# Janspiry/Image-Super-Resolution-via-Iterative-Refinement

Measured on NVIDIA H100. Metric: diffusion steps/sec (batch16, 16->128 SR3), higher is better.
Workload: dtype bf16

## Files before the change

image-super-resolution-via-iterative-refinement_b200/csrc/attn_wgmma.cuh:

```cuda
#pragma once
#include <cuda_bf16.h>
#include <cuda.h>
#include "gemm_wgmma.cuh"

namespace sr3 {

constexpr int ATTN_THREADS = 288;
constexpr int ATTN_PRODUCER_WARP = 8;
constexpr int ATTN_STAGES = 3;
constexpr int ATTN_STAGE_BYTES = 16384 + 32768;
constexpr int ATTN_P_BYTES = 65536;
constexpr int ATTN_SMEM_BYTES = 1024 + GEMM_HDR_BYTES + ATTN_STAGES * ATTN_STAGE_BYTES + ATTN_P_BYTES;

struct AttnParams {
    CUtensorMap qk_map;
    CUtensorMap vt_map;
    __nv_bfloat16* out;
    int C, Lt, HW, dn, nz;
    float scale_log2e;
};

template <int LT, int DN>
__device__ __forceinline__ void attn_unit_t(const AttnParams& p, const AttnParams* pm, const uint32_t base_in, uint8_t* base_ptr_in,
                                            const int qt, const int dc, const int z) {
    const uint32_t bar_base = base_in;
    const uint32_t base = base_in + GEMM_HDR_BYTES;
    uint8_t* base_ptr = base_ptr_in + GEMM_HDR_BYTES;
    const uint32_t p_base = base + ATTN_STAGES * ATTN_STAGE_BYTES;
    uint8_t* p_ptr = base_ptr + ATTN_STAGES * ATTN_STAGE_BYTES;
    auto full_bar = [&](int s) { return bar_base + 8u * s; };
    auto empty_bar = [&](int s) { return bar_base + 8u * (ATTN_STAGES + s); };

    const int warp = threadIdx.x >> 5;
    const int lane = threadIdx.x & 31;
    const int kc1 = p.C / 64;
    constexpr int kc3 = LT / 64;

    if (threadIdx.x == 0) {
        tma_prefetch_desc(&pm->qk_map);
        tma_prefetch_desc(&pm->vt_map);
        for (int s = 0; s < ATTN_STAGES; ++s) { mbar_init(full_bar(s), 1); mbar_init(empty_bar(s), 2); }
        fence_mbar_init();
    }
    __syncthreads();
    pdl_launch_dependents();
    pdl_wait();

    if (warp == ATTN_PRODUCER_WARP) {
        int s = 0;
        uint32_t ph = 0;
        for (int it = 0; it < kc1 + kc3; ++it) {
            mbar_wait(empty_bar(s), ph ^ 1u);
            if (elect_one_sync()) {
                const uint32_t dst = base + s * ATTN_STAGE_BYTES;
                if (it < kc1) {
                    mbar_arrive_expect_tx(full_bar(s), 16384 + LT * 128);
                    tma_load_2d(dst, &pm->qk_map, full_bar(s), it * 64, z * LT + qt * 128);
                    for (int j = 0; j < LT / 128; ++j)
                        tma_load_2d(dst + 16384 + j * 16384, &pm->qk_map, full_bar(s), p.C + it * 64, z * LT + j * 128);
                } else {
                    mbar_arrive_expect_tx(full_bar(s), DN * 128);
                    for (int j = 0; j < DN / 128; ++j)
                        tma_load_2d(dst + 16384 + j * 16384, &pm->vt_map, full_bar(s), (it - kc1) * 64, z * p.C + dc * DN + j * 128);
                }
            }
            __syncwarp();
            if (++s == ATTN_STAGES) { s = 0; ph ^= 1u; }
        }
    } else if (warp < ATTN_PRODUCER_WARP) {
        const int g = warp >> 2;
        const int wq = warp & 3;
        const bool leader = (threadIdx.x & 127) == 0;
        int s = 0, prev = -1;
        uint32_t ph = 0;
        auto release_prev = [&]() {
            if (prev >= 0) {
                wgmma_wait<1>();
                mbar_arrive_if(empty_bar(prev), leader);
            }
            prev = s;
            if (++s == ATTN_STAGES) { s = 0; ph ^= 1u; }
        };
        float sacc[LT / 2];
        for (int it = 0; it < kc1; ++it) {
            mbar_wait(full_bar(s), ph);
            wgmma_fence();
            const uint32_t st = base + s * ATTN_STAGE_BYTES;
#pragma unroll
            for (int kk = 0; kk < 4; ++kk)
                Wgmma<LT>::template mma<0, 0>(sacc, wgmma_desc_sw128(st + g * 8192 + kk * 32, 16, 1024), wgmma_desc_sw128(st + 16384 + kk * 32, 16, 1024),
                                              (it | kk) != 0);
            wgmma_commit();
            release_prev();
        }
        wgmma_wait<0>();
        wgmma_fence_regs(sacc);
        int rows[2], segs[2];
        float mx[2] = {-3.0e38f, -3.0e38f}, sum[2] = {0.f, 0.f};
#pragma unroll
        for (int h = 0; h < 2; ++h) {
            rows[h] = 64 * g + 16 * wq + (lane >> 2) + 8 * h;
            segs[h] = (qt * 128 + rows[h]) / p.HW;
        }
#pragma unroll
        for (int j = 0; j < LT / 2; ++j) {
            const int h = (j >> 1) & 1, key = 8 * (j >> 2) + 2 * (lane & 3) + (j & 1);
            if (key / p.HW == segs[h]) mx[h] = fmaxf(mx[h], sacc[j]);
        }
#pragma unroll
        for (int h = 0; h < 2; ++h) {
            mx[h] = fmaxf(mx[h], __shfl_xor_sync(0xffffffffu, mx[h], 1));
            mx[h] = fmaxf(mx[h], __shfl_xor_sync(0xffffffffu, mx[h], 2));
        }
        const float mxs[2] = {mx[0] * p.scale_log2e, mx[1] * p.scale_log2e};
#pragma unroll
        for (int j = 0; j < LT / 2; j += 2) {
            const int h = (j >> 1) & 1, key = 8 * (j >> 2) + 2 * (lane & 3);
            const float x0 = exp2f(fmaf(sacc[j], p.scale_log2e, -mxs[h])), x1 = exp2f(fmaf(sacc[j + 1], p.scale_log2e, -mxs[h]));
            const float e0 = (key / p.HW == segs[h]) ? x0 : 0.f, e1 = ((key + 1) / p.HW == segs[h]) ? x1 : 0.f;
            sum[h] += e0 + e1;
            const int r = rows[h];
            uint8_t* dst = p_ptr + (key >> 6) * 16384 + (r >> 3) * 1024 + (r & 7) * 128 + ((((key & 63) >> 3) ^ (r & 7)) << 4) + (key & 7) * 2;
            *reinterpret_cast<__nv_bfloat162*>(dst) = __floats2bfloat162_rn(e0, e1);
        }
#pragma unroll
        for (int h = 0; h < 2; ++h) {
            sum[h] += __shfl_xor_sync(0xffffffffu, sum[h], 1);
            sum[h] += __shfl_xor_sync(0xffffffffu, sum[h], 2);
        }
        fence_proxy_async_smem();
        asm volatile("bar.sync %0, 128;" ::"r"(2 + g) : "memory");

        float oacc[DN / 2];
        for (int kc = 0; kc < kc3; ++kc) {
            mbar_wait(full_bar(s), ph);
            wgmma_fence();
            const uint32_t st = base + s * ATTN_STAGE_BYTES;
            const uint32_t pa = p_base + kc * 16384 + g * 8192;
#pragma unroll
            for (int kk = 0; kk < 4; ++kk)
                Wgmma<DN>::template mma<0, 0>(oacc, wgmma_desc_sw128(pa + kk * 32, 16, 1024), wgmma_desc_sw128(st + 16384 + kk * 32, 16, 1024),
                                              (kc | kk) != 0);
            wgmma_commit();
            release_prev();
        }
        wgmma_wait<0>();
        wgmma_fence_regs(oacc);
        if (prev >= 0) mbar_arrive_if(empty_bar(prev), leader);
        const float inv[2] = {1.0f / sum[0], 1.0f / sum[1]};
#pragma unroll
        for (int j = 0; j < DN / 2; j += 2) {
            const int h = (j >> 1) & 1, col = 8 * (j >> 2) + 2 * (lane & 3);
            __nv_bfloat16* o = p.out + (static_cast<long long>(z) * LT + qt * 128 + rows[h]) * p.C + dc * DN + col;
            *reinterpret_cast<__nv_bfloat162*>(o) = __floats2bfloat162_rn(oacc[j] * inv[h], oacc[j + 1] * inv[h]);
        }
    }
    __syncthreads();
}

__device__ __forceinline__ void attn_unit(const AttnParams& p, const AttnParams* pm, const uint32_t base, uint8_t* base_ptr, const int qt,
                                          const int dc, const int z) {
    if (p.Lt == 256) {
        if (p.dn == 256) attn_unit_t<256, 256>(p, pm, base, base_ptr, qt, dc, z);
        else attn_unit_t<256, 128>(p, pm, base, base_ptr, qt, dc, z);
    } else {
        if (p.dn == 256) attn_unit_t<128, 256>(p, pm, base, base_ptr, qt, dc, z);
        else attn_unit_t<128, 128>(p, pm, base, base_ptr, qt, dc, z);
    }
}

__global__ void __launch_bounds__(ATTN_THREADS, 1) attn_kernel(const __grid_constant__ AttnParams p) {
    extern __shared__ uint8_t smem_raw[];
    const uint32_t raw = smem_u32(smem_raw);
    const uint32_t base = (raw + 1023u) & ~1023u;
    const int n_dc = p.C / p.dn;
    attn_unit(p, &p, base, smem_raw + (base - raw), blockIdx.x / n_dc, blockIdx.x % n_dc, blockIdx.y);
}

}
```

image-super-resolution-via-iterative-refinement_b200/csrc/engine.cu:

```cuda
#include <cuda.h>
#include <cuda_runtime.h>

#include <cmath>
#include <cstdarg>
#include <cstdlib>
#include <cstring>
#include <functional>
#include <limits>
#include <map>
#include <memory>
#include <mutex>
#include <stdexcept>
#include <string>
#include <vector>

#include "../../include/sr3_b200.h"
#include "aux_kernels.cuh"
#include "attn_wgmma.cuh"
#include "attn_long_wgmma.cuh"
#include "train_kernels.cuh"
#include "window_kernels.cuh"
#include "stream_kernels.cuh"

using namespace sr3;
// ... 122 lines not shown
    if (s < 1) s = 1;
    return s;
}
int current_device() { int dev = 0; CK(cudaGetDevice(&dev)); return dev; }
int num_sms() {
    static std::map<int, int> cache;
    static std::mutex mu;
    std::lock_guard<std::mutex> lock(mu);
    const int dev = current_device();
    auto it = cache.find(dev);
    if (it != cache.end()) return it->second;
    int n = 0;
    CK(cudaDeviceGetAttribute(&n, cudaDevAttrMultiProcessorCount, dev));
    cache[dev] = n;
    return n;
}
bool first_use_on_device(std::vector<int>& seen) {
    static std::mutex mu;
    std::lock_guard<std::mutex> lock(mu);
    const int dev = current_device();
    for (int d : seen) if (d == dev) return false;
    seen.push_back(dev);
    return true;
}
template <typename... KArgs, typename... Args>
void launch_k(void (*kernel)(KArgs...), dim3 grid, dim3 block, size_t smem, cudaStream_t st, Args&&... args) {
    cudaLaunchConfig_t cfg{};
    cfg.gridDim = grid; cfg.blockDim = block; cfg.dynamicSmemBytes = smem; cfg.stream = st;
    cudaLaunchAttribute attr[1];
    attr[0].id = cudaLaunchAttributeProgrammaticStreamSerialization;
    attr[0].val.programmaticStreamSerializationAllowed = 1;
    cfg.attrs = attr; cfg.numAttrs = 1;
    CK(cudaLaunchKernelEx(&cfg, kernel, std::forward<Args>(args)...));
}
constexpr int MAX_CLUSTER_SPLIT = 8;
template <int BN, int MH, bool PP = false>
void launch_gemm_bn(const GemmParams& p, dim3 grid, int smem, cudaStream_t st) {
    if (p.ksplit == 1) { launch_k(gemm_tile_kernel<BN, MH, PP>, grid, dim3(GEMM_THREADS), (size_t)smem, st, p); return; }
    REQUIRE(!PP, "a ping-pong tile launch cannot be split");
    REQUIRE(p.ksplit <= MAX_CLUSTER_SPLIT && grid.x % p.ksplit == 0, "split-K factor %d does not form clusters of grid %u", p.ksplit, grid.x);
    cudaLaunchConfig_t cfg{};
    cfg.gridDim = grid; cfg.blockDim = dim3(GEMM_THREADS); cfg.dynamicSmemBytes = (size_t)smem; cfg.stream = st;
    cudaLaunchAttribute attr[2];
    attr[0].id = cudaLaunchAttributeClusterDimension;
    attr[0].val.clusterDim.x = (unsigned)p.ksplit; attr[0].val.clusterDim.y = 1; attr[0].val.clusterDim.z = 1;
    attr[1].id = cudaLaunchAttributeProgrammaticStreamSerialization;
    attr[1].val.programmaticStreamSerializationAllowed = 1;
    cfg.attrs = attr; cfg.numAttrs = 2;
    CK(cudaLaunchKernelEx(&cfg, gemm_tile_kernel<BN, MH>, p));
}
void init_gemm_attrs() {
    static std::vector<int> seen;
    if (!first_use_on_device(seen)) return;
    CK(cudaFuncSetAttribute(gemm_tile_kernel<16, 1>, cudaFuncAttributeMaxDynamicSharedMemorySize, SMEM_LIMIT));
    CK(cudaFuncSetAttribute(gemm_tile_kernel<16, 2>, cudaFuncAttributeMaxDynamicSharedMemorySize, SMEM_LIMIT));
    CK(cudaFuncSetAttribute(gemm_tile_kernel<32, 1>, cudaFuncAttributeMaxDynamicSharedMemorySize, SMEM_LIMIT));
    CK(cudaFuncSetAttribute(gemm_tile_kernel<64, 1>, cudaFuncAttributeMaxDynamicSharedMemorySize, SMEM_LIMIT));
    CK(cudaFuncSetAttribute(gemm_tile_kernel<64, 2>, cudaFuncAttributeMaxDynamicSharedMemorySize, SMEM_LIMIT));
    CK(cudaFuncSetAttribute(gemm_tile_kernel<128, 1>, cudaFuncAttributeMaxDynamicSharedMemorySize, SMEM_LIMIT));
    CK(cudaFuncSetAttribute(gemm_tile_kernel<128, 2>, cudaFuncAttributeMaxDynamicSharedMemorySize, SMEM_LIMIT));
    CK(cudaFuncSetAttribute(gemm_tile_kernel<256, 1>, cudaFuncAttributeMaxDynamicSharedMemorySize, SMEM_LIMIT));
    CK(cudaFuncSetAttribute(gemm_tile_kernel<64, 2, true>, cudaFuncAttributeMaxDynamicSharedMemorySize, SMEM_LIMIT));
    CK(cudaFuncSetAttribute(gemm_tile_kernel<64, 1, true>, cudaFuncAttributeMaxDynamicSharedMemorySize, SMEM_LIMIT));
    CK(cudaFuncSetAttribute(gemm_tile_kernel<128, 1, true>, cudaFuncAttributeMaxDynamicSharedMemorySize, SMEM_LIMIT));
}

int cluster_capacity(int c) {
    static std::map<std::pair<int, int>, int> cache;
    static std::mutex mu;
    if (c <= 1) return num_sms();
    init_gemm_attrs();
    std::lock_guard<std::mutex> lock(mu);
    const std::pair<int, int> key(current_device(), c);
    auto it = cache.find(key);
    if (it != cache.end()) return it->second;
    cudaLaunchConfig_t cfg{};
    cfg.gridDim = dim3(c * 32); cfg.blockDim = dim3(GEMM_THREADS); cfg.dynamicSmemBytes = SMEM_LIMIT;
    cudaLaunchAttribute attr[1];
    attr[0].id = cudaLaunchAttributeClusterDimension;
    attr[0].val.clusterDim.x = (unsigned)c; attr[0].val.clusterDim.y = 1; attr[0].val.clusterDim.z = 1;
    cfg.attrs = attr; cfg.numAttrs = 1;
    int n = 0;
    if (cudaOccupancyMaxActiveClusters(&n, gemm_tile_kernel<64, 1>, &cfg) != cudaSuccess || n <= 0) {
        cudaGetLastError();
        n = 8 * ((num_sms() / 8) / c);
    }
    cache[key] = n;
    return n;
}
int fit_split(int want, long long tiles) {
    if (want > MAX_CLUSTER_SPLIT) want = MAX_CLUSTER_SPLIT;
    while (want > 1 && cluster_capacity(want) < tiles) --want;
    return want;
}

struct DevAllocs {
    std::vector<void*> ptrs;
    long long bytes = 0;
    void* alloc(size_t n, bool zero = true) {
        void* p = nullptr;
        if (n == 0) n = 16;
        CK(cudaMalloc(&p, n));
        if (zero) CK(cudaMemset(p, 0, n));
        ptrs.push_back(p);
        bytes += (long long)n;
        return p;
    }
    ~DevAllocs() { for (void* p : ptrs) cudaFree(p); }
};

typedef std::function<void(cudaStream_t)> Op;
struct GemmHandle { std::shared_ptr<GemmParams> p; const void* w_ptr = nullptr; long long w_bytes = 0; bool w_is_param = false; int bn = 0, mh = 0; };
static thread_local std::vector<GemmHandle>* g_gemm_registry = nullptr;
struct LastTestConv { sr3_gemm_geometry geo{}; int schedule = -1; int out_hwc[3] = {0, 0, 0}; };
static thread_local LastTestConv g_last_test_conv;

Op make_gemm_op(const GemmDesc& d, DevAllocs& mem, sr3_gemm_geometry* geo = nullptr, int* schedule = nullptr) {
    REQUIRE(d.w_box * d.h_box * d.b_box == 128 * d.mh, "tile box must cover %d rows", 128 * d.mh);
    REQUIRE(!d.slabs.empty(), "gemm without K slabs");
    GemmParams p;
    memset(&p, 0, sizeof(p));
    const int abw = d.a_box_w ? d.a_box_w : d.w_box, abh = d.a_box_h ? d.a_box_h : d.h_box, abb = d.a_box_b ? d.a_box_b : d.b_box;
    p.a_stage_bytes = abw * abh * abb * 128;
    REQUIRE(p.a_stage_bytes % 1024 == 0, "A box must be a whole number of swizzle atoms");
    for (int i = 0; i < 2; ++i) {
        const ASrc& a = d.a[i < d.n_a ? i : 0];
        REQUIRE(a.C % 64 == 0, "A channels (%d) must be a multiple of 64", a.C);
        const uint64_t dims[5] = {(uint64_t)a.C, (uint64_t)a.W, (uint64_t)a.P, (uint64_t)a.H, (uint64_t)a.Bn};
        const uint64_t str[4] = {(uint64_t)a.sW, (uint64_t)a.sP, (uint64_t)a.sH, (uint64_t)a.sB};
        const uint32_t box[5] = {64u, (uint32_t)abw, 1u, (uint32_t)abh, (uint32_t)abb};
        p.a_map[i] = encode_map(5, a.ptr, dims, str, box);
    }
    {
        REQUIRE(d.b_K % 64 == 0, "B K extent must be a multiple of 64");
        const uint64_t dims[2] = {(uint64_t)d.b_K, (uint64_t)d.b_rows};
        const uint64_t str[1] = {2ull * d.b_K};
        const uint32_t box[2] = {64u, (uint32_t)d.block_n};
        REQUIRE(d.b_rows >= d.block_n, "B rows %lld < block_n %d", d.b_rows, d.block_n);
        p.b_map = encode_map(2, d.b_ptr, dims, str, box);
    }
    std::vector<StageDesc> tab;
    int b_taps = 1, a_boxes = 1;
    for (size_t i = 0; i < d.slabs.size(); ++i) {
        const KSlab& k = d.slabs[i];
        REQUIRE(k.a_sel < d.n_a, "slab refers to missing A source");
        StageDesc e; memset(&e, 0, sizeof(e));
        e.a_sel = k.a_sel; e.ntaps = 1;
        e.tap[0].a_chan = k.a_chan; e.tap[0].dw = k.dw; e.tap[0].dh = k.dh; e.tap[0].p = k.p; e.tap[0].b_col = k.b_col;
        if (d.tall) {
            bool first = true;
            int nt = 0;
            for (const KSlab& o : d.slabs) {
                if (o.a_sel != k.a_sel || o.a_chan != k.a_chan || o.dw != k.dw) continue;
                if (&o < &k) { first = false; break; }
                REQUIRE(nt < 3 && o.p == 0 && o.dh >= -1 && o.dh <= 1, "bad tall tap group");
                e.tap[nt] = e.tap[0];
                e.tap[nt].dh = -1;
                e.tap[nt].b_col = o.b_col;
                e.tap[nt].a_off = (o.dh + 1) * 1024;
                ++nt;
            }
            if (!first) continue;
            e.ntaps = nt;
            if (nt > b_taps) b_taps = nt;
        } else {
            e.a_multi = 1;
            int n = 1;
            while (n < 3 && i + n < d.slabs.size() && d.slabs[i + n].a_sel == k.a_sel) ++n;
            e.ntaps = n;
            for (int t = 0; t < n; ++t) {
                const KSlab& o = d.slabs[i + t];
                e.tap[t].a_chan = o.a_chan; e.tap[t].dw = o.dw; e.tap[t].dh = o.dh; e.tap[t].p = o.p; e.tap[t].b_col = o.b_col;
                e.tap[t].a_off = t * p.a_stage_bytes;
            }
            if (n > b_taps) b_taps = n;
            if (n > a_boxes) a_boxes = n;
            i += n - 1;
        }
        tab.push_back(e);
    }
    p.a_box_bytes = p.a_stage_bytes;
    p.a_stage_bytes = p.a_box_bytes * a_boxes;
    REQUIRE((int)tab.size() <= GEMM_MAX_K, "gemm with %d stages per tile (max %d)", (int)tab.size(), GEMM_MAX_K);
    StageDesc* dtab = static_cast<StageDesc*>(mem.alloc(tab.size() * sizeof(StageDesc), false));
    CK(cudaMemcpy(dtab, tab.data(), tab.size() * sizeof(StageDesc), cudaMemcpyHostToDevice));
    p.ktab = dtab; p.num_k = (int)tab.size();
    p.b_taps = b_taps; p.a_half_off = d.a_half_off;
    p.tiles_w = d.tiles_w; p.tiles_h = d.tiles_h; p.tiles_b = d.tiles_b;
    p.w_box = d.w_box; p.h_box = d.h_box; p.b_box = d.b_box;
    {
        auto lg = [](int v) { int l = 0; while ((1 << l) < v) ++l; return l; };
        REQUIRE((d.w_box & (d.w_box - 1)) == 0 && (d.h_box & (d.h_box - 1)) == 0, "tile box %dx%d must be powers of two", d.w_box, d.h_box);
        p.w_shift = lg(d.w_box); p.h_shift = lg(d.h_box);
    }
    p.a_zstep = d.a_zstep; p.b_zrows = d.b_zrows;
    p.n_tiles = d.n_tiles; p.nz = d.nz;
    p.mode = d.mode; p.OW = d.OW; p.OH = d.OH; p.OB = d.OB; p.n_valid = d.n_valid; p.scale = d.scale;
    p.bias = d.bias; p.bias2 = d.bias2; p.bias2_stride = d.bias2_stride;
    p.resid = d.resid; p.rs = d.rs; p.out_f32 = d.out_f32; p.os = d.os; p.out_bf16 = d.out_bf16; p.hs = d.hs;
    p.out_t = d.out_t; p.t_col0 = d.t_col0; p.t_rows = d.t_rows; p.t_ld = d.t_ld; p.t_per = d.t_per > 0 ? d.t_per : 1;
    p.stats = d.stats; p.stats_C = d.stats_C; p.stats_coff = d.stats_coff; p.ctl = d.ctl; p.post = d.post;
    p.z_phase = d.z_phase; p.z_off_hi = d.z_off_hi; p.z_off_lo = d.z_off_lo;
    p.passes = d.passes; p.lo_b_col = d.lo_b_col; p.lo_a_chan[0] = d.lo_a_chan[0]; p.lo_a_chan[1] = d.lo_a_chan[1];
    p.lo_out_off = d.lo_out_off; p.lo_t_off = d.lo_t_off;
    if (d.stats) REQUIRE((d.w_box * d.h_box) % 32 == 0, "stats need whole warps per image");
    p.tma_epi = (d.mode == 0 && (d.out_f32 || d.resid)) ? 1 : 0;
    if (p.tma_epi) {
        const int w_sub = d.w_box < 32 ? d.w_box : 32, h_sub = 32 / w_sub;
        REQUIRE(d.w_box % w_sub == 0 && (d.h_box % h_sub == 0 || d.h_box == 1) && (h_sub == 1 || (128 / w_sub) % h_sub == 0), "tile box %dx%d cannot be split into per-warp boxes", d.w_box, d.h_box);
        auto mk = [&](const float* ptr, const OutSpec& o, bool& c4z) {
            c4z = (o.sB == 0 && o.sZ != 0);
            const long long s4 = c4z ? o.sZ : o.sB;
            const uint64_t n4 = c4z ? (uint64_t)d.nz : d.out_imgs ? (uint64_t)d.out_imgs : (uint64_t)(d.tiles_b * d.b_box > d.OB ? d.tiles_b * d.b_box : d.OB);
            uint64_t dims[5] = {(uint64_t)d.n_valid, (uint64_t)d.OW, 1ull, (uint64_t)d.OH, n4};
            uint64_t str[4];
            str[0] = (uint64_t)o.sW * 4;
            str[1] = str[0] * d.OW;
            str[2] = d.OH > 1 ? (uint64_t)o.sH * 4 : str[1];
            str[3] = s4 != 0 ? (uint64_t)s4 * 4 : str[2] * d.OH;
            if (d.z_phase) {
                REQUIRE(d.z_off_lo == d.n_valid && o.sW == 2 * d.n_valid, "phase-batched output must be NHWC with 2x the width");
                dims[0] = 2ull * d.n_valid; dims[2] = 2ull; str[1] = (uint64_t)d.z_off_hi * 4;
            }
            const uint32_t box[5] = {32u, (uint32_t)w_sub, 1u, (uint32_t)h_sub, 1u};
            REQUIRE(d.n_valid >= 32, "TMA epilogue needs at least 32 output columns");
            return encode_map(5, ptr + o.off, dims, str, box, CU_TENSOR_MAP_DATA_TYPE_FLOAT32);
        };
        bool zo = false, zr = false;
        if (d.out_f32) p.out_map = mk(d.out_f32, d.os, zo);
        if (d.resid) p.res_map = mk(d.resid, d.rs, zr);
        if (d.out_f32 && d.resid) REQUIRE(zo == zr, "output and residual must share the batch coordinate");
        if (!d.out_f32) p.out_map = p.res_map;
        if (!d.resid) p.res_map = p.out_map;
        p.epi_c4_is_z = (d.out_f32 ? zo : zr) ? 1 : 0;
    } else {
        p.out_map = p.b_map; p.res_map = p.b_map;
    }
    p.ksplit = 1;
    {
        const int tiles = d.tiles_w * d.tiles_h * d.tiles_b * d.n_tiles * d.nz;
        const int ks = d.ksplit_max;
        if (ks > 1 && !d.pingpong && d.mode == 0 && d.out_f32 && d.block_n >= 32 && d.n_valid % 32 == 0) {
            int want = num_sms() / tiles;
            if (want > ks) want = ks;
            if (want > p.num_k * d.passes / 2) want = p.num_k * d.passes / 2;
            const int units = d.mh * (d.block_n / 32) * 4;
            if (want > units) want = units;
            want = fit_split(want, tiles);
            if (want > 1) {
                p.ksplit = want;
                p.ws = static_cast<float*>(mem.alloc((size_t)tiles * want * d.mh * 128 * d.block_n * sizeof(float), false));
                p.counters = static_cast<unsigned int*>(mem.alloc((size_t)tiles * sizeof(unsigned int)));
            }
        }
    }
    const int total_tiles = d.tiles_w * d.tiles_h * d.tiles_b * d.n_tiles * d.nz * p.ksplit;
    int ctas = total_tiles < num_sms() ? total_tiles : num_sms();
    if (const char* e = getenv("SR3_MAX_CTAS")) { int v = atoi(e); if (v > 0 && v < ctas) ctas = v; }
    REQUIRE(p.ksplit == 1 || ctas == total_tiles, "split-K launch needs one CTA per (tile, split) pair: %d CTAs for %d (SR3_MAX_CTAS with a split tile)", ctas, total_tiles);
    const dim3 grid(ctas, 1, 1);
    const int bn = d.block_n;
    const int mh = d.mh;
    const bool res_smem = p.tma_epi && d.resid != nullptr && p.ksplit <= 1;
    p.stages = pick_stages(d.block_n, p.a_stage_bytes, p.b_taps, res_smem, p.num_k);
    const int smem = gemm_smem_bytes(bn, p.a_stage_bytes, p.b_taps, p.stages, res_smem, p.num_k);
    REQUIRE(smem <= SMEM_LIMIT, "gemm shared memory %d exceeds the limit", smem);
    init_gemm_attrs();
    REQUIRE((bn == 16 || bn == 32 || bn == 64 || bn == 128 || bn == 256) && (mh == 1 || (mh == 2 && bn <= 128 && bn != 32)), "unsupported tile %dx%d", 128 * mh, bn);
    const bool pp = d.pingpong != 0;
    REQUIRE(!pp || (gemm_pingpong_ok(bn, mh) && p.ksplit == 1 && d.mode == 0), "no ping-pong form of tile %dx%d (split %d)", 128 * mh, bn, p.ksplit);
    if (geo) {
        geo->tall = d.tall; geo->mh = mh; geo->block_n = bn; geo->h_box = d.h_box; geo->b_box = d.b_box;
        geo->ksplit = p.ksplit; geo->stages = p.stages; geo->ctas = ctas; geo->tiles = total_tiles / p.ksplit; geo->res_smem = res_smem ? 1 : 0;
    }
    if (schedule) *schedule = pp ? 1 : 0;
    std::shared_ptr<GemmParams> sp = std::make_shared<GemmParams>(p);
    if (g_gemm_registry) {
        GemmHandle h; h.p = sp; h.w_ptr = d.b_ptr; h.w_bytes = 2LL * d.b_rows * d.b_K; h.w_is_param = d.b_is_param; h.bn = bn; h.mh = mh;
        g_gemm_registry->push_back(h);
    }
    return [sp, grid, bn, mh, pp, smem](cudaStream_t st) {
        const GemmParams& p = *sp;
        if (pp) {
            if (mh == 2) launch_gemm_bn<64, 2, true>(p, grid, smem, st);
            else if (bn == 64) launch_gemm_bn<64, 1, true>(p, grid, smem, st);
            else launch_gemm_bn<128, 1, true>(p, grid, smem, st);
            return;
        }
        switch (bn) {
            case 16: if (mh == 2) launch_gemm_bn<16, 2>(p, grid, smem, st); else launch_gemm_bn<16, 1>(p, grid, smem, st); break;
            case 32: launch_gemm_bn<32, 1>(p, grid, smem, st); break;
            case 64: if (mh == 2) launch_gemm_bn<64, 2>(p, grid, smem, st); else launch_gemm_bn<64, 1>(p, grid, smem, st); break;
            case 128: if (mh == 2) launch_gemm_bn<128, 2>(p, grid, smem, st); else launch_gemm_bn<128, 1>(p, grid, smem, st); break;
            default: launch_gemm_bn<256, 1>(p, grid, smem, st); break;
        }
    };
}

bool attn_fusable(int Lt, int C) { return Lt >= 128 && Lt % 128 == 0 && C % 128 == 0 && C >= 128; }

Op make_attn_op(const bf16* qk, const bf16* vT, bf16* out, int nz, int Lt, int HW, int C) {
    REQUIRE(attn_fusable(Lt, C) && Lt % HW == 0, "attention shape Lt=%d HW=%d C=%d is not supported by the fused kernel", Lt, HW, C);
    REQUIRE(Lt <= 256 || HW == Lt, "attention over %d tokens per batch takes one image per batch (HW=%d)", Lt, HW);
    AttnParams p;
    memset(&p, 0, sizeof(p));
    {
        const uint64_t dims[2] = {(uint64_t)2 * C, (uint64_t)nz * Lt};
        const uint64_t str[1] = {(uint64_t)2 * C * 2};
        const uint32_t box[2] = {64u, 128u};
        p.qk_map = encode_map(2, qk, dims, str, box);
    }
    {
        const uint64_t dims[2] = {(uint64_t)Lt, (uint64_t)nz * C};
        const uint64_t str[1] = {(uint64_t)Lt * 2};
        const uint32_t box[2] = {64u, 128u};
        p.vt_map = encode_map(2, vT, dims, str, box);
    }
    p.out = out; p.C = C; p.Lt = Lt; p.HW = HW; p.nz = nz;
    p.dn = (C % 256 == 0) ? 256 : 128;
    p.scale_log2e = 1.4426950408889634f / sqrtf((float)C);
    if (Lt > 256) {
        p.dn = ATTNL_DN;
        static std::vector<int> seen_long;
        if (first_use_on_device(seen_long)) CK(cudaFuncSetAttribute(attn_long_kernel, cudaFuncAttributeMaxDynamicSharedMemorySize, ATTNL_SMEM_BYTES));
        const dim3 grid((Lt / 128) * (C / ATTNL_DN), nz, 1);
        return [p, grid](cudaStream_t st) { launch_k(attn_long_kernel, grid, dim3(ATTN_THREADS), ATTNL_SMEM_BYTES, st, p); };
    }
    static std::vector<int> seen;
    if (first_use_on_device(seen)) CK(cudaFuncSetAttribute(attn_kernel, cudaFuncAttributeMaxDynamicSharedMemorySize, ATTN_SMEM_BYTES));
    const dim3 grid((Lt / 128) * (C / p.dn), nz, 1);
    return [p, grid](cudaStream_t st) { launch_k(attn_kernel, grid, dim3(ATTN_THREADS), ATTN_SMEM_BYTES, st, p); };
}

void pick_image_box(int W, int H, int& w_box, int& h_box, int& b_box);
int pick_block_n(int cout);
int pingpong_knob() {
    const char* e = getenv("SR3_PINGPONG");
    return e ? (atoi(e) != 0 ? 1 : 0) : -1;
}

void conv_geometry(GemmDesc& d, int OW, int OH, int Bt, int cout, bool has_resid = false, int nz = 1) {
    const int npass = d.passes > 1 ? d.passes : 1;
    bool tall_ok = OW >= 8 && OH >= 16, has3 = false;
    for (const KSlab& k : d.slabs) { if (k.p != 0) tall_ok = false; if (k.dh != 0) has3 = true; }
    tall_ok = tall_ok && has3 && (OH >= 32 || Bt % 2 == 0);
    const int sms = num_sms();
    const int pp_knob = pingpong_knob();
    const bool pp_force = pp_knob == 1, pp_auto = pp_knob < 0;
    const bool shape_forced = getenv("SR3_TALL_BN") || getenv("SR3_TALL_MH") || getenv("SR3_BLOCK_N");
    constexpr double EPI_COOP = 200000.0, EPI_COOP_256x128 = 2000000.0, EPI_PP_128REG = 600000.0;
    const double EPI_PP_64REG = tall_ok ? 200000.0 : 10000.0;
    auto items_of = [](int rows, int bn) { return (double)(rows / 128) * (bn >= 32 ? bn / 32 : 1); };
    auto model = [&](long long tiles, int nstage, long long stage_bytes, int rows, int bn, int& split, bool pp = false) -> double {
        if (pp) {
            split = 1;
            const long long t = (tiles + sms - 1) / sms;
            const double mma = (double)nstage * stage_bytes, epi = items_of(rows, bn) * (rows == 128 && bn == 64 ? EPI_PP_64REG : EPI_PP_128REG);
            const double serial = (double)t * mma + epi, paired = (double)((t + 1) / 2) * (mma + epi);
            return serial > paired ? serial : paired;
        }
        int smax = 1;
        if (bn >= 32 && cout % 32 == 0) {
            smax = (int)(sms / tiles);
            const int units = (rows / 128) * (bn / 32) * 4;
            if (smax > units) smax = units;
            if (smax > nstage / 2) smax = nstage / 2;
            if (smax > 16) smax = 16;
            if (smax < 1) smax = 1;
            smax = fit_split(smax, tiles);
        }
        split = smax;
        const long long waves = (tiles * smax + sms - 1) / sms;
        double c = (double)waves * ((nstage + smax - 1) / smax) * (double)stage_bytes;
        const double warps = gemm_single_wg(bn, rows / 128) ? 4.0 : 8.0;
        c += (double)waves * items_of(rows, bn) * 4.0 / (warps * smax) * (rows == 256 && bn == 128 ? EPI_COOP_256x128 : EPI_COOP);
        if (smax > 1) c += 4.0 * rows * bn * 4 + 2000000.0 + (has_resid ? 2.0 * rows * bn * 4 : 0.0);
        return c;
    };
    d.ksplit_max = 1;
    if (tall_ok) {
        d.tall = 1; d.w_box = 8;
        struct Cand { int mh, bn; };
        const Cand cands[4] = {{2, 128}, {2, 64}, {1, 64}, {1, 32}};
        auto geom = [&](int mh, int& h_box, int& b_box) {
            if (mh == 2 && OH >= 32) { h_box = 32; b_box = 1; }
            else if (mh == 2) { h_box = 16; b_box = 2; }
            else { h_box = 16; b_box = 1; }
        };
        int nstage = 0;
        for (size_t i = 0; i < d.slabs.size(); ++i) {
            bool first = true;
            for (size_t j = 0; j < i; ++j)
                if (d.slabs[j].a_sel == d.slabs[i].a_sel && d.slabs[j].a_chan == d.slabs[i].a_chan && d.slabs[j].dw == d.slabs[i].dw) { first = false; break; }
            if (first) ++nstage;
        }
        int mh = 2, bn = 16, split = 1, pp = 0;
        if (cout % 32 == 0) {
            double best = 1e300, best_pp = 1e300;
            int pp_mh = 0, pp_bn = 0;
            for (int i = 0; i < 4; ++i) {
                const Cand& c = cands[i];
                if (cout % c.bn != 0) continue;
                int hb, bb; geom(c.mh, hb, bb);
                const long long tiles = (long long)(OW / 8) * (OH / hb) * ((Bt + bb - 1) / bb) * (cout / c.bn) * nz;
                const long long stage_bytes = (c.mh == 2 ? 36864 : 18432) + 3ll * c.bn * 128;
                int sp = 1;
                const double cost = model(tiles, nstage * npass, stage_bytes, c.mh * 128, c.bn, sp);
                if (gemm_pingpong_ok(c.bn, c.mh)) {
                    int sp1 = 1;
                    const double cpp = model(tiles, nstage * npass, stage_bytes, c.mh * 128, c.bn, sp1, true);
                    if (cpp < best_pp) { best_pp = cpp; pp_mh = c.mh; pp_bn = c.bn; }
                }
                if (c.bn == 128 && has_resid && sp <= 1) continue;
                if (cost < best) { best = cost; mh = c.mh; bn = c.bn; split = sp; }
            }
            if (!shape_forced && pp_bn && (pp_force || (pp_auto && best_pp < best))) { mh = pp_mh; bn = pp_bn; split = 1; pp = 1; }
        }
        if (const char* e = getenv("SR3_TALL_BN")) { int v = atoi(e); if ((v == 32 || v == 64 || v == 128) && cout % v == 0) { bn = v; split = 16; } }
        if (const char* e = getenv("SR3_TALL_MH")) { int v = atoi(e); if (v == 1 || v == 2) { mh = v; split = 16; } }
        if (mh == 2 && bn == 32) bn = 64;
        if (shape_forced) pp = (pp_force && gemm_pingpong_ok(bn, mh)) ? 1 : 0;
        if (pp) split = 1;
        d.mh = mh; d.block_n = bn; d.ksplit_max = split; d.pingpong = pp;
        geom(mh, d.h_box, d.b_box);
        d.a_box_w = 8; d.a_box_b = d.b_box;
        if (mh == 2 && d.b_box == 1) { d.a_box_h = 34; d.a_half_off = 16 * 1024; }
        else if (mh == 2) { d.a_box_h = 18; d.a_half_off = 18 * 1024; }
        else { d.a_box_h = 18; d.a_half_off = 0; }
    } else {
        d.tall = 0; d.mh = 1;
        pick_image_box(OW, OH, d.w_box, d.h_box, d.b_box);
        d.block_n = pick_block_n(cout);
        const long long mt = (long long)(OW / d.w_box) * ((OH + d.h_box - 1) / d.h_box) * ((Bt + d.b_box - 1) / d.b_box) * nz;
        if (getenv("SR3_BLOCK_N") == nullptr && cout % 32 == 0) {
            const int nstage = (((int)d.slabs.size() + 2) / 3) * npass;
            double best = 1e300, best_pp = 1e300;
            int pp_bn = 0;
            for (int bn = 128; bn >= 32; bn >>= 1) {
                if (cout % bn != 0) continue;
                int sp = 1;
                const long long tiles = mt * (cout / bn);
                const double cost = model(tiles, nstage, 3ll * (16384 + bn * 128), 128, bn, sp);
                if (gemm_pingpong_ok(bn, 1) && gemm_smem_bytes(bn, 3 * 16384, 3, 2, has_resid, nstage / npass) <= SMEM_LIMIT) {
                    int sp1 = 1;
                    const double cpp = model(tiles, nstage, 3ll * (16384 + bn * 128), 128, bn, sp1, true);
                    if (cpp < best_pp) { best_pp = cpp; pp_bn = bn; }
                }
                if (bn == 128 && sp > 1) continue;
                if (cost < best) { best = cost; d.block_n = bn; d.ksplit_max = sp; }
            }
            if (pp_bn && (pp_force || (pp_auto && best_pp < best))) { d.block_n = pp_bn; d.ksplit_max = 1; d.pingpong = 1; }
        } else if (pp_force && gemm_pingpong_ok(d.block_n, 1)) {
            d.pingpong = 1;
        }
    }
    if (d.pingpong) d.ksplit_max = 1;
    if (const char* e = getenv("SR3_KSPLIT")) d.ksplit_max = atoi(e);
    d.tiles_w = OW / d.w_box; d.tiles_h = (OH + d.h_box - 1) / d.h_box; d.tiles_b = (Bt + d.b_box - 1) / d.b_box;
}

void pick_image_box(int W, int H, int& w_box, int& h_box, int& b_box) {
    w_box = W < 16 ? W : 16;
    h_box = 128 / w_box;
    if (h_box > H) h_box = H;
    if (w_box * h_box < 32) h_box = 32 / w_box;
    b_box = 128 / (w_box * h_box);
}

int pick_block_n(int cout) {
    if (const char* e = getenv("SR3_BLOCK_N")) { int v = atoi(e); if (v == 32 || v == 64 || v == 128 || v == 256) if (cout % v == 0) return v; }
    if (cout % 128 == 0) return 128;
    if (cout % 64 == 0) return 64;
    return 16;
}

void add_conv_slabs(std::vector<KSlab>& slabs, int a_sel, int cin, int ksize, int stride, int b_col0, int row = 0) {
    if (row == 0) row = cin;
    if (ksize == 1) {
        for (int c = 0; c < cin; c += 64) slabs.push_back({a_sel, c, 0, 0, 0, b_col0 + c});
        return;
    }
    for (int r = 0; r < 3; ++r)
        for (int s = 0; s < 3; ++s)
            for (int c = 0; c < cin; c += 64) {
                KSlab k; k.a_sel = a_sel; k.b_col = b_col0 + (r * 3 + s) * cin + c;
                if (stride == 1) { k.dh = r - 1; k.dw = s - 1; k.p = 0; k.a_chan = c; }
                else {
                    k.dh = (r == 0) ? -1 : 0; k.p = (r == 1) ? 0 : 1;
                    k.dw = (s == 0) ? -1 : 0; k.a_chan = ((s == 1) ? 0 : row) + c;
                }
                slabs.push_back(k);
            }
}

struct Act {
    float* p = nullptr; double* stats = nullptr;
    int C = 0, H = 0, W = 0;
    float* g = nullptr; bf16* gb = nullptr; float* gsum = nullptr;
};

struct ParamEntry {
    std::string name;
    std::vector<int64_t> shape;
    int64_t numel = 0;
    bool loaded = false;
};

struct LayerSpec { std::string name; int kind; int cin, cout; bool attn; int res; };

void set_precise_fields(GemmDesc& d, int c0, int c1, int ktot) {
    d.passes = 3; d.lo_a_chan[0] = c0; d.lo_a_chan[1] = c1; d.lo_b_col = ktot;
}

struct ConvArgs {
    ASrc a[2]; int n_a = 1;
    std::vector<KSlab> slabs;
    const bf16* w = nullptr; int ktot = 0; int cout = 0;
    int OH = 0, OW = 0;
    const float* bias = nullptr; const float* bias2 = nullptr; int bias2_stride = 0;
    const float* resid = nullptr;
    Act out;
    bf16* raw_out = nullptr;
    bool custom_os = false; OutSpec os{};
    int nz = 1, b_zrows = 0, z_phase = 0; long long z_off_hi = 0, z_off_lo = 0;
    int c0 = 0, c1 = 0;
};

GemmDesc conv_desc(const ConvArgs& c, int B, int Bt, int PW) {
    GemmDesc d;
    d.n_a = c.n_a; d.a[0] = c.a[0]; d.a[1] = c.a[1];
    d.slabs = c.slabs;
    REQUIRE(PW == 1 || c.c0 > 0, "precise mode: conv without source channel counts");
    REQUIRE(!(c.raw_out && c.custom_os), "a bf16 copy of a phase-addressed (folded upsample) output is not supported");
    if (PW == 2) set_precise_fields(d, c.c0, c.c1, c.ktot);
    conv_geometry(d, c.OW, c.OH, Bt, c.cout, c.resid != nullptr, c.nz);
    d.b_ptr = c.w; d.b_K = PW * c.ktot; d.b_rows = (long long)c.nz * (((c.cout + 127) / 128) * 128);
    d.b_is_param = true;
    d.n_tiles = (c.cout + d.block_n - 1) / d.block_n; d.nz = c.nz; d.a_zstep = 0; d.b_zrows = c.b_zrows;
    d.z_phase = c.z_phase; d.z_off_hi = c.z_off_hi; d.z_off_lo = c.z_off_lo;
    d.OW = c.OW; d.OH = c.OH; d.OB = B; d.n_valid = c.cout;
    d.bias = c.bias; d.bias2 = c.bias2; d.bias2_stride = c.bias2_stride;
    d.resid = c.resid; d.rs = nhwc_out(c.OH, c.OW, c.cout);
    d.out_f32 = c.out.p; d.os = c.custom_os ? c.os : nhwc_out(c.OH, c.OW, c.cout);
    if (c.raw_out) { d.out_bf16 = c.raw_out; d.hs = nhwc_out(c.OH, c.OW, PW * c.cout); d.lo_out_off = PW == 2 ? c.cout : 0; }
    d.stats = c.out.stats; d.stats_C = c.cout; d.stats_coff = 0;
    return d;
}

void fold_up_conv(ConvArgs& c, const bf16* raw, int Bp, int Hl, int Wl, int C, int PW) {
    c.n_a = 1; c.a[0] = nhwc_src(raw, Bp, Hl, Wl, C * PW); c.c0 = C;
    for (int a = 0; a < 2; ++a)
        for (int bb = 0; bb < 2; ++bb)
            for (int ch = 0; ch < C; ch += 64) {
                KSlab k; k.a_sel = 0; k.a_chan = ch; k.dh = a - 1; k.dw = bb - 1; k.p = 0; k.b_col = (a * 2 + bb) * C + ch;
                c.slabs.push_back(k);
            }
    c.ktot = 4 * C; c.cout = C; c.OH = Hl; c.OW = Wl;
    c.custom_os = true;
    c.os.sZ = 0; c.os.sB = 4LL * Hl * Wl * C; c.os.sH = 4LL * Wl * C; c.os.sW = 2LL * C; c.os.off = 0;
    c.nz = 4; c.b_zrows = ((C + 127) / 128) * 128; c.z_phase = 1; c.z_off_hi = 2LL * Wl * C; c.z_off_lo = C;
}

std::vector<WgradTap> taps_3x3() {
    std::vector<WgradTap> t;
    for (int r = 0; r < 3; ++r) for (int s = 0; s < 3; ++s) t.push_back({0, s - 1, 0, r - 1});
    return t;
}
std::vector<WgradTap> taps_1x1() { return {{0, 0, 0, 0}}; }
std::vector<WgradTap> taps_3x3_stride2(int C) {
    std::vector<WgradTap> t;
    for (int r = 0; r < 3; ++r) for (int s = 0; s < 3; ++s) t.push_back({(s == 1) ? 0 : C, (s == 0) ? -1 : 0, (r == 1) ? 0 : 1, (r == 0) ? -1 : 0});
    return t;
}

struct WgradOut { float* ptr = nullptr; long long slice_stride = 0, row_stride = 0; int nb = 0; };

struct WgradShape { int co_pad = 0, tpc = 0, nx = 0, ny = 0, patches = 0, slices = 0; };
int wgrad_grid(int extent) { return extent == 4 ? 8 : extent; }
WgradShape wgrad_shape(int CY, int OHh, int OWw, int nbatch, int Cin, int ntaps, int slices, const WgradOut* raw) {
    OHh = wgrad_grid(OHh); OWw = wgrad_grid(OWw);
    REQUIRE(OHh % 8 == 0 && OWw % 8 == 0 && Cin % 64 == 0 && CY % 64 == 0, "wgrad geometry %dx%d Cin=%d CY=%d", OHh, OWw, Cin, CY);
    REQUIRE(ntaps >= 1 && ntaps <= WGRAD_MAX_TAPS, "too many taps");
    WgradShape s;
    s.co_pad = ((CY + 127) / 128) * 128;
    s.tpc = ntaps < 3 ? ntaps : 3;
    s.ny = (ntaps + s.tpc - 1) / s.tpc;
    s.nx = (s.co_pad / 128) * (Cin / 64);
    s.patches = nbatch * (OHh / 8) * (OWw / 8);
    if (raw) {
        s.slices = raw->nb;
    } else if (slices > 0) {
        REQUIRE(slices <= s.patches, "%d slices of %d patches", slices, s.patches);
        s.slices = slices;
    } else {
        const int nxy = s.nx * s.ny;
        s.slices = (num_sms() + nxy / 2) / nxy;
        if (s.slices > s.patches / 2) s.slices = s.patches / 2;
        if (s.slices < 1) s.slices = 1;
    }
    return s;
}
WgradParams wgrad_params(const WgradShape& s, const bf16* dy, int CY, int OHh, int OWw, int nmap, int nbatch, const ASrc& xs, int Cin,
                         const std::vector<WgradTap>& taps, int cout_valid, float* ws, const WgradOut* raw) {
    WgradParams p; memset(&p, 0, sizeof(p));
    const int ntaps = (int)taps.size();
    {
        const uint64_t dims[5] = {(uint64_t)CY, (uint64_t)OWw, 1ull, (uint64_t)OHh, (uint64_t)nmap};
        const uint64_t str[4] = {2ull * CY, 2ull * OWw * CY, 2ull * OWw * CY, 2ull * OHh * OWw * CY};
        const uint32_t box[5] = {64u, 8u, 1u, 8u, 1u};
        p.dy_map = encode_map(5, dy, dims, str, box);
    }
    {
        const uint64_t dims[5] = {(uint64_t)xs.C, (uint64_t)xs.W, (uint64_t)xs.P, (uint64_t)xs.H, (uint64_t)xs.Bn};
        const uint64_t str[4] = {(uint64_t)xs.sW, (uint64_t)xs.sP, (uint64_t)xs.sH, (uint64_t)xs.sB};
        const uint32_t box[5] = {64u, 8u, 1u, 8u, 1u};
        p.x_map = encode_map(5, xs.ptr, dims, str, box);
    }
    p.ws = ws; p.Cin = Cin; p.co_pad = s.co_pad; p.cout_valid = cout_valid;
    p.ws_slice_stride = raw ? raw->slice_stride : (long long)s.co_pad * ntaps * Cin; p.ws_row_stride = raw ? raw->row_stride : (long long)ntaps * Cin;
    p.OH = wgrad_grid(OHh); p.OW = wgrad_grid(OWw); p.B = nbatch; p.ntaps = ntaps; p.taps_per_cta = s.tpc; p.patches = s.patches; p.slices = s.slices;
    for (int i = 0; i < ntaps; ++i) p.taps[i] = taps[i];
    return p;
}
WgradReduceDesc wgrad_reduce_desc(const WgradShape& s, const float* ws, int ntaps, int Cin, int cout_valid, int cin_valid) {
    const int sw = s.slices >= 8 ? 8 : (s.slices >= 4 ? 4 : (s.slices >= 2 ? 2 : 1));
    const int ci_per_block = 32 * (8 / sw);
    WgradReduceDesc rd{}; rd.ws = ws; rd.grad = nullptr; rd.slices = s.slices; rd.co_pad = s.co_pad; rd.ntaps = ntaps; rd.Cin = Cin; rd.cout_valid = cout_valid;
    rd.cin_valid = cin_valid; rd.sw = sw; rd.blocks_x = (cin_valid + ci_per_block - 1) / ci_per_block;
    return rd;
}
void pack_one(const PackDesc& d, cudaStream_t st) {
    pack_one_kernel<<<pack_entry_blocks(d), 256, 0, st>>>(d);
    CK(cudaGetLastError());
}
// ... 2421 lines not shown
```

Baseline: 140.9.

## Shrink short attention kernel to one 64-row consumer warpgroup with more CTAs

The short-sequence fused attention kernel goes from two consumer warpgroups over 128 query rows to one warpgroup over 64 query rows, with a 4-stage pipeline and smaller stage and P buffers. The grid doubles along the query axis, and the 256-wide output split is only chosen when there are more CTAs than SMs, so small attention layers fill more SMs. The kernel is now templated and launched directly instead of branching at runtime, and the segment test uses an unsigned range compare instead of integer division. In exchange, K and V tiles are reloaded for twice as many CTAs, and each CTA does less work to hide latency.

```diff
diff --git a/image-super-resolution-via-iterative-refinement_b200/csrc/attn_wgmma.cuh b/image-super-resolution-via-iterative-refinement_b200/csrc/attn_wgmma.cuh
--- a/image-super-resolution-via-iterative-refinement_b200/csrc/attn_wgmma.cuh
+++ b/image-super-resolution-via-iterative-refinement_b200/csrc/attn_wgmma.cuh
@@ -7,10 +7,13 @@
 
 constexpr int ATTN_THREADS = 288;
 constexpr int ATTN_PRODUCER_WARP = 8;
-constexpr int ATTN_STAGES = 3;
-constexpr int ATTN_STAGE_BYTES = 16384 + 32768;
-constexpr int ATTN_P_BYTES = 65536;
-constexpr int ATTN_SMEM_BYTES = 1024 + GEMM_HDR_BYTES + ATTN_STAGES * ATTN_STAGE_BYTES + ATTN_P_BYTES;
+
+constexpr int ATTN_S_THREADS = 160;
+constexpr int ATTN_S_PRODUCER_WARP = 4;
+constexpr int ATTN_S_STAGES = 4;
+constexpr int ATTN_S_STAGE_BYTES = 8192 + 32768;
+constexpr int ATTN_S_P_BYTES = 32768;
+constexpr int ATTN_S_SMEM_BYTES = 1024 + GEMM_HDR_BYTES + ATTN_S_STAGES * ATTN_S_STAGE_BYTES + ATTN_S_P_BYTES;
 
 struct AttnParams {
     CUtensorMap qk_map;
@@ -21,56 +24,59 @@
 };
 
 template <int LT, int DN>
-__device__ __forceinline__ void attn_unit_t(const AttnParams& p, const AttnParams* pm, const uint32_t base_in, uint8_t* base_ptr_in,
-                                            const int qt, const int dc, const int z) {
-    const uint32_t bar_base = base_in;
-    const uint32_t base = base_in + GEMM_HDR_BYTES;
-    uint8_t* base_ptr = base_ptr_in + GEMM_HDR_BYTES;
-    const uint32_t p_base = base + ATTN_STAGES * ATTN_STAGE_BYTES;
-    uint8_t* p_ptr = base_ptr + ATTN_STAGES * ATTN_STAGE_BYTES;
+__global__ void __launch_bounds__(ATTN_S_THREADS, 1) attn_kernel(const __grid_constant__ AttnParams p) {
+    extern __shared__ uint8_t smem_raw[];
+    const uint32_t raw = smem_u32(smem_raw);
+    const uint32_t bar_base = (raw + 1023u) & ~1023u;
+    const uint32_t base = bar_base + GEMM_HDR_BYTES;
+    const uint32_t p_base = base + ATTN_S_STAGES * ATTN_S_STAGE_BYTES;
+    uint8_t* p_ptr = smem_raw + (p_base - raw);
     auto full_bar = [&](int s) { return bar_base + 8u * s; };
-    auto empty_bar = [&](int s) { return bar_base + 8u * (ATTN_STAGES + s); };
+    auto empty_bar = [&](int s) { return bar_base + 8u * (ATTN_S_STAGES + s); };
 
+    const int n_dc = p.C / DN;
+    const int qt = blockIdx.x / n_dc, dc = blockIdx.x % n_dc, z = blockIdx.y;
     const int warp = threadIdx.x >> 5;
     const int lane = threadIdx.x & 31;
     const int kc1 = p.C / 64;
     constexpr int kc3 = LT / 64;
 
     if (threadIdx.x == 0) {
-        tma_prefetch_desc(&pm->qk_map);
-        tma_prefetch_desc(&pm->vt_map);
-        for (int s = 0; s < ATTN_STAGES; ++s) { mbar_init(full_bar(s), 1); mbar_init(empty_bar(s), 2); }
+        tma_prefetch_desc(&p.qk_map);
+        tma_prefetch_desc(&p.vt_map);
+        for (int s = 0; s < ATTN_S_STAGES; ++s) { mbar_init(full_bar(s), 1); mbar_init(empty_bar(s), 1); }
         fence_mbar_init();
     }
     __syncthreads();
     pdl_launch_dependents();
     pdl_wait();
 
-    if (warp == ATTN_PRODUCER_WARP) {
+    if (warp == ATTN_S_PRODUCER_WARP) {
         int s = 0;
         uint32_t ph = 0;
         for (int it = 0; it < kc1 + kc3; ++it) {
             mbar_wait(empty_bar(s), ph ^ 1u);
             if (elect_one_sync()) {
-                const uint32_t dst = base + s * ATTN_STAGE_BYTES;
+                const uint32_t dst = base + s * ATTN_S_STAGE_BYTES;
                 if (it < kc1) {
-                    mbar_arrive_expect_tx(full_bar(s), 16384 + LT * 128);
-                    tma_load_2d(dst, &pm->qk_map, full_bar(s), it * 64, z * LT + qt * 128);
-                    for (int j = 0; j < LT / 128; ++j)
-                        tma_load_2d(dst + 16384 + j * 16384, &pm->qk_map, full_bar(s), p.C + it * 64, z * LT + j * 128);
+                    mbar_arrive_expect_tx(full_bar(s), 8192 + LT * 128);
+                    tma_load_2d(dst, &p.qk_map, full_bar(s), it * 64, z * LT + qt * 64);
+#pragma unroll
+                    for (int j = 0; j < LT / 64; ++j)
+                        tma_load_2d(dst + 8192 + j * 8192, &p.qk_map, full_bar(s), p.C + it * 64, z * LT + j * 64);
                 } else {
                     mbar_arrive_expect_tx(full_bar(s), DN * 128);
+#pragma unroll
                     for (int j = 0; j < DN / 128; ++j)
-                        tma_load_2d(dst + 16384 + j * 16384, &pm->vt_map, full_bar(s), (it - kc1) * 64, z * p.C + dc * DN + j * 128);
+                        tma_load_2d(dst + 8192 + j * 16384, &p.vt_map, full_bar(s), (it - kc1) * 64, z * p.C + dc * DN + j * 128);
                 }
             }
             __syncwarp();
-            if (++s == ATTN_STAGES) { s = 0; ph ^= 1u; }
+            if (++s == ATTN_S_STAGES) { s = 0; ph ^= 1u; }
         }
-    } else if (warp < ATTN_PRODUCER_WARP) {
-        const int g = warp >> 2;
-        const int wq = warp & 3;
-        const bool leader = (threadIdx.x & 127) == 0;
+    } else if (warp < ATTN_S_PRODUCER_WARP) {
+        const int wq = warp;
+        const bool leader = threadIdx.x == 0;
         int s = 0, prev = -1;
         uint32_t ph = 0;
         auto release_prev = [&]() {
@@ -79,33 +85,34 @@
                 mbar_arrive_if(empty_bar(prev), leader);
             }
             prev = s;
-            if (++s == ATTN_STAGES) { s = 0; ph ^= 1u; }
+            if (++s == ATTN_S_STAGES) { s = 0; ph ^= 1u; }
         };
         float sacc[LT / 2];
         for (int it = 0; it < kc1; ++it) {
             mbar_wait(full_bar(s), ph);
             wgmma_fence();
-            const uint32_t st = base + s * ATTN_STAGE_BYTES;
+            const uint32_t st = base + s * ATTN_S_STAGE_BYTES;
 #pragma unroll
             for (int kk = 0; kk < 4; ++kk)
-                Wgmma<LT>::template mma<0, 0>(sacc, wgmma_desc_sw128(st + g * 8192 + kk * 32, 16, 1024), wgmma_desc_sw128(st + 16384 + kk * 32, 16, 1024),
+                Wgmma<LT>::template mma<0, 0>(sacc, wgmma_desc_sw128(st + kk * 32, 16, 1024), wgmma_desc_sw128(st + 8192 + kk * 32, 16, 1024),
                                               (it | kk) != 0);
             wgmma_commit();
             release_prev();
         }
         wgmma_wait<0>();
         wgmma_fence_regs(sacc);
-        int rows[2], segs[2];
+        int rows[2], k_lo[2];
         float mx[2] = {-3.0e38f, -3.0e38f}, sum[2] = {0.f, 0.f};
 #pragma unroll
         for (int h = 0; h < 2; ++h) {
-            rows[h] = 64 * g + 16 * wq + (lane >> 2) + 8 * h;
-            segs[h] = (qt * 128 + rows[h]) / p.HW;
+            rows[h] = 16 * wq + (lane >> 2) + 8 * h;
+            k_lo[h] = (qt * 64 + rows[h]) / p.HW * p.HW;
         }
+        auto in_seg = [&](int key, int h) { return static_cast<unsigned>(key - k_lo[h]) < static_cast<unsigned>(p.HW); };
 #pragma unroll
         for (int j = 0; j < LT / 2; ++j) {
             const int h = (j >> 1) & 1, key = 8 * (j >> 2) + 2 * (lane & 3) + (j & 1);
-            if (key / p.HW == segs[h]) mx[h] = fmaxf(mx[h], sacc[j]);
+            if (in_seg(key, h)) mx[h] = fmaxf(mx[h], sacc[j]);
         }
 #pragma unroll
         for (int h = 0; h < 2; ++h) {
@@ -117,10 +124,10 @@
         for (int j = 0; j < LT / 2; j += 2) {
             const int h = (j >> 1) & 1, key = 8 * (j >> 2) + 2 * (lane & 3);
             const float x0 = exp2f(fmaf(sacc[j], p.scale_log2e, -mxs[h])), x1 = exp2f(fmaf(sacc[j + 1], p.scale_log2e, -mxs[h]));
-            const float e0 = (key / p.HW == segs[h]) ? x0 : 0.f, e1 = ((key + 1) / p.HW == segs[h]) ? x1 : 0.f;
+            const float e0 = in_seg(key, h) ? x0 : 0.f, e1 = in_seg(key + 1, h) ? x1 : 0.f;
             sum[h] += e0 + e1;
             const int r = rows[h];
-            uint8_t* dst = p_ptr + (key >> 6) * 16384 + (r >> 3) * 1024 + (r & 7) * 128 + ((((key & 63) >> 3) ^ (r & 7)) << 4) + (key & 7) * 2;
+            uint8_t* dst = p_ptr + (key >> 6) * 8192 + (r >> 3) * 1024 + (r & 7) * 128 + ((((key & 63) >> 3) ^ (r & 7)) << 4) + (key & 7) * 2;
             *reinterpret_cast<__nv_bfloat162*>(dst) = __floats2bfloat162_rn(e0, e1);
         }
 #pragma unroll
@@ -129,17 +136,17 @@
             sum[h] += __shfl_xor_sync(0xffffffffu, sum[h], 2);
         }
         fence_proxy_async_smem();
-        asm volatile("bar.sync %0, 128;" ::"r"(2 + g) : "memory");
+        asm volatile("bar.sync 1, 128;" ::: "memory");
 
         float oacc[DN / 2];
         for (int kc = 0; kc < kc3; ++kc) {
             mbar_wait(full_bar(s), ph);
             wgmma_fence();
-            const uint32_t st = base + s * ATTN_STAGE_BYTES;
-            const uint32_t pa = p_base + kc * 16384 + g * 8192;
+            const uint32_t st = base + s * ATTN_S_STAGE_BYTES;
+            const uint32_t pa = p_base + kc * 8192;
 #pragma unroll
             for (int kk = 0; kk < 4; ++kk)
-                Wgmma<DN>::template mma<0, 0>(oacc, wgmma_desc_sw128(pa + kk * 32, 16, 1024), wgmma_desc_sw128(st + 16384 + kk * 32, 16, 1024),
+                Wgmma<DN>::template mma<0, 0>(oacc, wgmma_desc_sw128(pa + kk * 32, 16, 1024), wgmma_desc_sw128(st + 8192 + kk * 32, 16, 1024),
                                               (kc | kk) != 0);
             wgmma_commit();
             release_prev();
@@ -151,30 +158,10 @@
 #pragma unroll
         for (int j = 0; j < DN / 2; j += 2) {
             const int h = (j >> 1) & 1, col = 8 * (j >> 2) + 2 * (lane & 3);
-            __nv_bfloat16* o = p.out + (static_cast<long long>(z) * LT + qt * 128 + rows[h]) * p.C + dc * DN + col;
+            __nv_bfloat16* o = p.out + (static_cast<long long>(z) * LT + qt * 64 + rows[h]) * p.C + dc * DN + col;
             *reinterpret_cast<__nv_bfloat162*>(o) = __floats2bfloat162_rn(oacc[j] * inv[h], oacc[j + 1] * inv[h]);
         }
     }
-    __syncthreads();
-}
-
-__device__ __forceinline__ void attn_unit(const AttnParams& p, const AttnParams* pm, const uint32_t base, uint8_t* base_ptr, const int qt,
-                                          const int dc, const int z) {
-    if (p.Lt == 256) {
-        if (p.dn == 256) attn_unit_t<256, 256>(p, pm, base, base_ptr, qt, dc, z);
-        else attn_unit_t<256, 128>(p, pm, base, base_ptr, qt, dc, z);
-    } else {
-        if (p.dn == 256) attn_unit_t<128, 256>(p, pm, base, base_ptr, qt, dc, z);
-        else attn_unit_t<128, 128>(p, pm, base, base_ptr, qt, dc, z);
-    }
-}
-
-__global__ void __launch_bounds__(ATTN_THREADS, 1) attn_kernel(const __grid_constant__ AttnParams p) {
-    extern __shared__ uint8_t smem_raw[];
-    const uint32_t raw = smem_u32(smem_raw);
-    const uint32_t base = (raw + 1023u) & ~1023u;
-    const int n_dc = p.C / p.dn;
-    attn_unit(p, &p, base, smem_raw + (base - raw), blockIdx.x / n_dc, blockIdx.x % n_dc, blockIdx.y);
 }
 
 }
diff --git a/image-super-resolution-via-iterative-refinement_b200/csrc/engine.cu b/image-super-resolution-via-iterative-refinement_b200/csrc/engine.cu
--- a/image-super-resolution-via-iterative-refinement_b200/csrc/engine.cu
+++ b/image-super-resolution-via-iterative-refinement_b200/csrc/engine.cu
@@ -448,12 +448,13 @@
 Op make_attn_op(const bf16* qk, const bf16* vT, bf16* out, int nz, int Lt, int HW, int C) {
     REQUIRE(attn_fusable(Lt, C) && Lt % HW == 0, "attention shape Lt=%d HW=%d C=%d is not supported by the fused kernel", Lt, HW, C);
     REQUIRE(Lt <= 256 || HW == Lt, "attention over %d tokens per batch takes one image per batch (HW=%d)", Lt, HW);
+    const bool long_form = Lt > 256;
     AttnParams p;
     memset(&p, 0, sizeof(p));
     {
         const uint64_t dims[2] = {(uint64_t)2 * C, (uint64_t)nz * Lt};
         const uint64_t str[1] = {(uint64_t)2 * C * 2};
-        const uint32_t box[2] = {64u, 128u};
+        const uint32_t box[2] = {64u, long_form ? 128u : 64u};
         p.qk_map = encode_map(2, qk, dims, str, box);
     }
     {
@@ -463,19 +464,23 @@
         p.vt_map = encode_map(2, vT, dims, str, box);
     }
     p.out = out; p.C = C; p.Lt = Lt; p.HW = HW; p.nz = nz;
-    p.dn = (C % 256 == 0) ? 256 : 128;
     p.scale_log2e = 1.4426950408889634f / sqrtf((float)C);
-    if (Lt > 256) {
+    if (long_form) {
         p.dn = ATTNL_DN;
         static std::vector<int> seen_long;
         if (first_use_on_device(seen_long)) CK(cudaFuncSetAttribute(attn_long_kernel, cudaFuncAttributeMaxDynamicSharedMemorySize, ATTNL_SMEM_BYTES));
         const dim3 grid((Lt / 128) * (C / ATTNL_DN), nz, 1);
         return [p, grid](cudaStream_t st) { launch_k(attn_long_kernel, grid, dim3(ATTN_THREADS), ATTNL_SMEM_BYTES, st, p); };
     }
+    p.dn = (C % 256 == 0 && (Lt / 64) * (C / 128) * nz > num_sms()) ? 256 : 128;
+    void (*kernel)(AttnParams) = Lt == 256 ? (p.dn == 256 ? attn_kernel<256, 256> : attn_kernel<256, 128>)
+                                           : (p.dn == 256 ? attn_kernel<128, 256> : attn_kernel<128, 128>);
     static std::vector<int> seen;
-    if (first_use_on_device(seen)) CK(cudaFuncSetAttribute(attn_kernel, cudaFuncAttributeMaxDynamicSharedMemorySize, ATTN_SMEM_BYTES));
-    const dim3 grid((Lt / 128) * (C / p.dn), nz, 1);
-    return [p, grid](cudaStream_t st) { launch_k(attn_kernel, grid, dim3(ATTN_THREADS), ATTN_SMEM_BYTES, st, p); };
+    if (first_use_on_device(seen))
+        for (auto k : {attn_kernel<256, 256>, attn_kernel<256, 128>, attn_kernel<128, 256>, attn_kernel<128, 128>})
+            CK(cudaFuncSetAttribute(k, cudaFuncAttributeMaxDynamicSharedMemorySize, ATTN_S_SMEM_BYTES));
+    const dim3 grid((Lt / 64) * (C / p.dn), nz, 1);
+    return [p, grid, kernel](cudaStream_t st) { launch_k(kernel, grid, dim3(ATTN_S_THREADS), ATTN_S_SMEM_BYTES, st, p); };
 }
 
 void pick_image_box(int W, int H, int& w_box, int& h_box, int& b_box);
```

Result: faster. 144.8, median of 6 (+2.7%).
